# krullgit/3D-Object-Detection-for-autonomous-navigation

Hardware: AMD Instinct MI355X
Metric: frames/sec (whole node) + p50 per-frame ms, 16k-pt pillars (higher is better)
Workload: dtype f32 (GEMMs on the 16-bit matrix pipe as split operands -- two float16 pieces per value, 3 products, fp32 accumulate: fp32-equivalent results, measured 1.5e-6 max from the fp32 oracle at this shape)

## Files before the change

### 3d-object-detection-for-autonomous-navigation_amd/csrc/pfn.hip

```cpp
#include <stdlib.h>

#include "pp_common.h"
#include "anchor_mask_dev.h"

template <int N>
struct FVec { float v[N]; };

__device__ __forceinline__ float bcast(float x, int srclane) {
    return __int_as_float(__builtin_amdgcn_readlane(__float_as_int(x), srclane));
}

__device__ __forceinline__ float raw_max(float a, float b) {
    float r;
    asm("v_max_f32 %0, %1, %2" : "=v"(r) : "v"(a), "v"(b));
    return r;
}

__device__ __forceinline__ float wave_sum(float x) {
#pragma unroll
    for (int off = 32; off >= 1; off >>= 1) x += __shfl_xor(x, off);
    return x;
}

#define PFN_CW 4
template <int CPL, int F, bool PADDED, bool DIST = false>
__global__ __launch_bounds__(256) void k_pfn_canvas(PfnParams p) {
    constexpr int FA = F + 5 + (DIST ? 1 : 0);
    const int lane = threadIdx.x & 63, wave = threadIdx.x >> 6;
    const int b = blockIdx.y;
    const int ncanvas = p.ny * p.nx;
    const int cell0 = (blockIdx.x * 4 + wave) * PFN_CW;
    if (cell0 >= ncanvas) return;
    const int ncells = min(PFN_CW, ncanvas - cell0);
    const int C = p.C;
    const int ch0 = lane * CPL;
    const bool ch_ok = ch0 < C;

    float w[FA][CPL], bias[CPL];
#pragma unroll
    for (int k = 0; k < FA; ++k)
#pragma unroll
        for (int q = 0; q < CPL; ++q) w[k][q] = ch_ok ? p.w[k * C + ch0 + q] : 0.f;
#pragma unroll
    for (int q = 0; q < CPL; ++q) bias[q] = ch_ok ? p.bias[ch0 + q] : 0.f;
    float wsx[CPL], wsy[CPL], wsz[CPL];
#pragma unroll
    for (int q = 0; q < CPL; ++q) {
        wsx[q] = (w[0][q] + w[F + 0][q]) + w[F + 3][q];
        wsy[q] = (w[1][q] + w[F + 1][q]) + w[F + 4][q];
        wsz[q] = w[2][q] + w[F + 2][q];
    }

    const int* map = p.cellmap + (size_t)b * p.nz * ncanvas;
    unsigned occ = 0;
    for (int z = 0; z < p.nz; ++z) {
        const int v = (lane < ncells) ? map[(size_t)z * ncanvas + cell0 + lane] : -1;
        occ |= (unsigned)(__ballot(v >= 0) & ((1ull << PFN_CW) - 1ull));
    }

    float* cbase = p.canvas + ((size_t)b * ncanvas + cell0) * C;
    {
        const int nq = ncells * C / 4;
        const float4 z4 = make_float4(0.f, 0.f, 0.f, 0.f);
        for (int q = lane; q < nq; q += 64) {
            const int c = (q * 4) / C;
            if (!((occ >> c) & 1u)) reinterpret_cast<float4*>(cbase)[q] = z4;
        }
    }

    const int n0 = PADDED ? 0 : p.offsets[b];
    const int* ps = PADDED ? nullptr : p.pillar_start + (size_t)b * (p.max_voxels + 1);
    const int T = p.T;

    while (occ) {
        const int c = __builtin_ctz(occ);
        occ &= occ - 1;
        const int cell = cell0 + c;
        const int yi = cell / p.nx, xi = cell - yi * p.nx;
        const float cxf = __fadd_rn(__fmul_rn((float)xi, p.vx), p.x_off);
        const float cyf = __fadd_rn(__fmul_rn((float)yi, p.vy), p.y_off);
        float acc[CPL];
#pragma unroll
        for (int q = 0; q < CPL; ++q) acc[q] = 0.f;

        for (int z = 0; z < p.nz; ++z) {
            const int pid = __builtin_amdgcn_readfirstlane(map[(size_t)z * ncanvas + cell]);
            if (pid < 0) continue;
            int n, nsum;
            const float* src;
            if (PADDED) {
                n = __builtin_amdgcn_readfirstlane(min(max(p.num_points[pid], 0), T));
                nsum = T;
                src = p.voxels + (size_t)pid * T * F;
            } else {
                const int start = __builtin_amdgcn_readfirstlane(ps[pid]);
                n = __builtin_amdgcn_readfirstlane(min(ps[pid + 1] - start, T));
                nsum = n;
                src = p.pts_sorted + (size_t)(n0 + start) * F;
            }
            float sx = 0.f, sy = 0.f, sz = 0.f;
            for (int j0 = 0; j0 < nsum; j0 += 64) {
                const int j = j0 + lane;
                if (j < nsum) {
                    const float* q = src + (size_t)j * F;
                    sx += q[0]; sy += q[1]; sz += q[2];
                }
            }
            sx = wave_sum(sx); sy = wave_sum(sy); sz = wave_sum(sz);
            const float fn = (float)n;
            const float mx = sx / fn, my = sy / fn, mz = sz / fn;

            const float dxm = mx - cxf, dym = my - cyf;
            float kp[CPL], m[CPL];
#pragma unroll
            for (int q = 0; q < CPL; ++q) {
                float k0 = bias[q];
                k0 = fmaf(cxf, w[0][q], k0);
                k0 = fmaf(cyf, w[1][q], k0);
                k0 = fmaf(-dxm, w[F + 0][q], k0);
                k0 = fmaf(-dym, w[F + 1][q], k0);
                k0 = fmaf(-mz, w[F + 2][q], k0);
                kp[q] = k0;
                m[q] = -3.0e38f;
            }
            for (int j0 = 0; j0 < n; j0 += 64) {
                const int j = j0 + lane;
                float pt[F];
#pragma unroll
                for (int f = 0; f < F; ++f) pt[f] = 0.f;
                if (j < n) {
                    const float* q = src + (size_t)j * F;
#pragma unroll
                    for (int f = 0; f < F; ++f) pt[f] = q[f];
                }
                float pdist = 0.f;
                if (DIST) pdist = __fsqrt_rn(__fadd_rn(__fadd_rn(__fmul_rn(pt[0], pt[0]), __fmul_rn(pt[1], pt[1])), __fmul_rn(pt[2], pt[2])));
                pt[0] = pt[0] - cxf;
                pt[1] = pt[1] - cyf;
                const int cnt = min(64, n - j0);
                for (int jj = 0; jj < cnt; ++jj) {
                    float ft[F];
#pragma unroll
                    for (int f = 0; f < F; ++f) ft[f] = bcast(pt[f], jj);
                    const float fd = DIST ? bcast(pdist, jj) : 0.f;
#pragma unroll
                    for (int q = 0; q < CPL; ++q) {
                        float o = kp[q];
                        o = fmaf(ft[0], wsx[q], o);
                        o = fmaf(ft[1], wsy[q], o);
                        o = fmaf(ft[2], wsz[q], o);
                        if (F > 3) o = fmaf(ft[F - 1], w[F - 1][q], o);
                        if (DIST) o = fmaf(fd, w[FA - 1][q], o);
                        m[q] = fmaxf(m[q], o);
                    }
                }
            }
#pragma unroll
            for (int q = 0; q < CPL; ++q) m[q] = fmaxf(m[q], 0.f);
            if (n < T) {
#pragma unroll
                for (int q = 0; q < CPL; ++q) m[q] = fmaxf(m[q], fmaxf(bias[q], 0.f));
            }
            if (p.feat_out != nullptr && ch_ok) {
                const size_t row = PADDED ? (size_t)pid : ((size_t)b * p.max_voxels + pid);
#pragma unroll
                for (int q = 0; q < CPL; ++q) p.feat_out[row * C + ch0 + q] = m[q];
            }
#pragma unroll
            for (int q = 0; q < CPL; ++q) acc[q] += m[q];
        }
        if (ch_ok) {
            float* dst = cbase + (size_t)c * C + ch0;
            if constexpr (CPL == 4) {
                *reinterpret_cast<float4*>(dst) = make_float4(acc[0], acc[1], acc[2], acc[3]);
            } else if constexpr (CPL == 2) {
                *reinterpret_cast<float2*>(dst) = make_float2(acc[0], acc[1]);
            } else {
                dst[0] = acc[0];
            }
        }
    }
}

#ifndef PFN2_CW
#define PFN2_CW 8
#endif
template <int CPL, int F, bool PIL = false>
__global__ __launch_bounds__(256) void k_pfn_canvas2(PfnParams p) {
    constexpr int FA = F + 5;
    const int lane = threadIdx.x & 63, wave = threadIdx.x >> 6;
    const int b = blockIdx.y;
    const int ncanvas = p.ny * p.nx;
    const int amb = (p.am_mask != nullptr) ? AM_PFN_BLOCKS : 0;
    if ((int)blockIdx.x < amb) {
        extern __shared__ int sI[];
        const int part = (int)blockIdx.x;
        const int64_t per = (p.am_A + AM_PFN_BLOCKS - 1) / AM_PFN_BLOCKS;
        const int64_t a0 = part * per, a1 = (a0 + per < p.am_A) ? a0 + per : p.am_A;
        anchor_mask_frame_block<256>(p.cellmap + (size_t)b * p.nz * ncanvas, p.nz, p.ny, p.nx, p.am_cells, a0, a1,
                                     p.am_threshold, p.am_mask + (size_t)b * p.am_A, sI);
        return;
    }
    const int bx = (int)blockIdx.x - amb;
    const int NW = PIL ? 1 : ((int)gridDim.x - amb) * 4;
    const int wid = PIL ? (bx * 4 + wave) * PFN2_CW : bx * 4 + wave;
    const int np_frame = PIL ? p.npillars[b] : 0;
    if (PIL ? (wid >= np_frame) : (wid >= ncanvas)) return;
    const int ncells = PIL ? min(PFN2_CW, np_frame - wid) : min(PFN2_CW, (ncanvas - wid + NW - 1) / NW);
    const int nz = p.nz;
    const int NS = ncells * nz;
    const int C = p.C, T = p.T;
    const int ch0 = lane * CPL;
    const bool ch_ok = ch0 < C;

    const int n0 = p.offsets[b];
    const int* ps = p.pillar_start + (size_t)b * (p.max_voxels + 1);
    int pid = -1, start = 0, cnt = 0, slot_cell = 0;
    float slot_cx = 0.f, slot_cy = 0.f;
    [[maybe_unused]] int col_xy = 0;
    if constexpr (PIL) {
        int z0 = 0;
        bool primary = false;
        if (lane < ncells) {
            const int cz = p.pillar_cell[(size_t)b * p.max_voxels + wid + lane];
            z0 = cz / ncanvas;
            col_xy = cz - z0 * ncanvas;
            primary = true;
            for (int z = 0; z < z0; ++z) primary = primary & (p.cellmap[((size_t)b * nz + z) * ncanvas + col_xy] < 0);
            if (p.occbits != nullptr) {
                const int yy = col_xy / p.nx, xx = col_xy - yy * p.nx;
                atomicOr(p.occbits + ((size_t)b * p.ny + yy) * occ_words(p.nx) + ((xx + 1) >> 6), 1ull << ((xx + 1) & 63));
            }
        }
        if (lane < NS) {
            const int c = lane / nz, z = lane - c * nz;
            slot_cell = c;
            const int cxy = __shfl(col_xy, c), zc = __shfl(z0, c);
            const bool prim = __shfl((int)primary, c) != 0;
            if (prim && z == zc) pid = wid + c;
            else if (prim && z > zc) pid = p.cellmap[((size_t)b * nz + z) * ncanvas + cxy];
        }
    } else {
        if (lane < NS) {
            const int c = lane / nz, z = lane - c * nz;
            slot_cell = c;
            pid = p.cellmap[((size_t)b * nz + z) * ncanvas + wid + c * NW];
        }
    }
    if (PIL && __ballot(pid >= 0) == 0ull) return;
    if (lane < NS) {
        const int c = slot_cell;
        if (pid >= 0) {
            start = ps[pid];
            cnt = min(ps[pid + 1] - start, T);
        }
        const int cell = PIL ? __shfl(col_xy, c) : wid + c * NW;
        const int yi = cell / p.nx, xi = cell - yi * p.nx;
        slot_cx = __fadd_rn(__fmul_rn((float)xi, p.vx), p.x_off);
        slot_cy = __fadd_rn(__fmul_rn((float)yi, p.vy), p.y_off);
    }
    float w[FA][CPL], bias[CPL];
#pragma unroll
    for (int k = 0; k < FA; ++k)
#pragma unroll
        for (int q = 0; q < CPL; ++q) w[k][q] = ch_ok ? p.w[k * C + ch0 + q] : 0.f;
#pragma unroll
    for (int q = 0; q < CPL; ++q) bias[q] = ch_ok ? p.bias[ch0 + q] : 0.f;
    float wsx[CPL], wsy[CPL], wsz[CPL];
#pragma unroll
    for (int q = 0; q < CPL; ++q) {
        wsx[q] = (w[0][q] + w[F + 0][q]) + w[F + 3][q];
        wsy[q] = (w[1][q] + w[F + 1][q]) + w[F + 4][q];
        wsz[q] = w[2][q] + w[F + 2][q];
    }

    const int incl = wave_inclusive_scan(cnt);
    const int excl = incl - cnt;
    const int tot = __builtin_amdgcn_readlane(incl, 63);
    if (PIL && tot == 0) return;
    const float* src = p.pts_sorted + (size_t)n0 * F;

    struct Batch { int slot; float x, y, z, i; };
    auto load_batch = [&](int base) -> Batch {
        Batch r;
        r.slot = -1; r.x = r.y = r.z = r.i = 0.f;
        const int g = base + lane;
        int sl = 0;
        for (int s = 0; s < NS; ++s) sl += (g >= __builtin_amdgcn_readlane(incl, s)) ? 1 : 0;
        sl = min(sl, NS - 1);
        const int st = __shfl(start, sl), ex = __shfl(excl, sl);
        const float pcx = __shfl(slot_cx, sl), pcy = __shfl(slot_cy, sl);
        if (g < tot) {
            r.slot = sl;
            const float* q = src + (size_t)(st + (g - ex)) * F;
            r.x = q[0] - pcx;
            r.y = q[1] - pcy;
            r.z = q[2];
            if (F > 3) r.i = q[F - 1];
        }
        return r;
    };

    float* cbase = p.canvas + ((size_t)b * ncanvas + (PIL ? 0 : wid)) * C;
    const size_t cstep = (size_t)NW * C;
    float acc[CPL], m[CPL];
#pragma unroll
    for (int q = 0; q < CPL; ++q) { acc[q] = 0.f; m[q] = -3.0e38f; }
    int cur_slot = -1, cur_cell = 0;
    float cxf = 0.f, cyf = 0.f, sx = 0.f, sy = 0.f, sz = 0.f;
    bool cell_dirty = false;
    auto write_cell = [&](int c) {
        if (ch_ok && (cell_dirty || !PIL)) {
            float* dst = PIL ? cbase + (size_t)__builtin_amdgcn_readlane(col_xy, c) * C + ch0 : cbase + (size_t)c * cstep + ch0;
            if constexpr (CPL == 4) *reinterpret_cast<float4*>(dst) = make_float4(acc[0], acc[1], acc[2], acc[3]);
            else if constexpr (CPL == 2) *reinterpret_cast<float2*>(dst) = make_float2(acc[0], acc[1]);
            else dst[0] = acc[0];
        }
#pragma unroll
        for (int q = 0; q < CPL; ++q) acc[q] = 0.f;
        cell_dirty = false;
    };
    auto finish_slot = [&](int s) {
        const int n = __builtin_amdgcn_readlane(cnt, s);
        const float rn = __builtin_amdgcn_rcpf((float)n);
        const float dxm = sx * rn, dym = sy * rn, mz = sz * rn;
#pragma unroll
        for (int q = 0; q < CPL; ++q) {
            float k0 = bias[q];
            k0 = fmaf(cxf, w[0][q], k0);
            k0 = fmaf(cyf, w[1][q], k0);
            k0 = fmaf(-dxm, w[F + 0][q], k0);
            k0 = fmaf(-dym, w[F + 1][q], k0);
            k0 = fmaf(-mz, w[F + 2][q], k0);
            m[q] = fmaxf(k0 + m[q], 0.f);
        }
        if (n < T) {
#pragma unroll
            for (int q = 0; q < CPL; ++q) m[q] = fmaxf(m[q], fmaxf(bias[q], 0.f));
        }
        if (p.feat_out != nullptr && ch_ok) {
            const size_t row = (size_t)b * p.max_voxels + __builtin_amdgcn_readlane(pid, s);
#pragma unroll
            for (int q = 0; q < CPL; ++q) p.feat_out[row * C + ch0 + q] = m[q];
        }
#pragma unroll
        for (int q = 0; q < CPL; ++q) { acc[q] += m[q]; m[q] = -3.0e38f; }
        cell_dirty = true;
    };
    auto begin_slot = [&](int s) {
        const int c = __builtin_amdgcn_readlane(slot_cell, s);
        while (cur_cell < c) { write_cell(cur_cell); ++cur_cell; }
        cxf = bcast(slot_cx, s);
        cyf = bcast(slot_cy, s);
        sx = sy = sz = 0.f;
        cur_slot = s;
    };
    Batch cur = load_batch(0);
    int left = 0;
    int next_slot = 0;
    for (int base = 0; base < tot; base += 64) {
        Batch nxt = cur;
        if (base + 64 < tot) nxt = load_batch(base + 64);
        const int nb = min(64, tot - base);
        for (int jj = 0; jj < nb; ++jj) {
            if (left == 0) {
                if (cur_slot >= 0) finish_slot(cur_slot);
                while ((left = __builtin_amdgcn_readlane(cnt, next_slot)) == 0) ++next_slot;
                begin_slot(next_slot);
                ++next_slot;
            }
            --left;
            const float fx = bcast(cur.x, jj), fy = bcast(cur.y, jj), fz = bcast(cur.z, jj);
            const float fi = (F > 3) ? bcast(cur.i, jj) : 0.f;
            sx += fx; sy += fy; sz += fz;
            if constexpr (CPL == 2) {
                typedef float f32x2 __attribute__((ext_vector_type(2)));
                const f32x2 vx = {fx, fx}, vy = {fy, fy}, vz = {fz, fz};
                const f32x2 wx2 = {wsx[0], wsx[1]}, wy2 = {wsy[0], wsy[1]}, wz2 = {wsz[0], wsz[1]};
                f32x2 o = vx * wx2;
                o = __builtin_elementwise_fma(vy, wy2, o);
                o = __builtin_elementwise_fma(vz, wz2, o);
                if (F > 3) {
                    const f32x2 vi = {fi, fi}, wi2 = {w[F - 1][0], w[F - 1][1]};
                    o = __builtin_elementwise_fma(vi, wi2, o);
                }
                m[0] = raw_max(m[0], o.x);
                m[1] = raw_max(m[1], o.y);
            } else {
#pragma unroll
                for (int q = 0; q < CPL; ++q) {
                    float o = fx * wsx[q];
                    o = fmaf(fy, wsy[q], o);
                    o = fmaf(fz, wsz[q], o);
                    if (F > 3) o = fmaf(fi, w[F - 1][q], o);
                    m[q] = raw_max(m[q], o);
                }
            }
        }
        cur = nxt;
    }
    if (cur_slot >= 0) finish_slot(cur_slot);
    while (cur_cell < ncells) { write_cell(cur_cell); ++cur_cell; }
}

static bool pfn_first_generation();
bool pfn_can_carry_anchor_mask(const PfnParams& p, bool padded_source) {
    return !padded_source && p.feat_out == nullptr && PFN2_CW * p.nz <= 64 && !pfn_first_generation() && !p.sparse &&
           p.ny * (p.nx | 1) <= AM_MAX_CELLS && !p.with_distance;
}
static bool pfn_first_generation() {
    static int v = -1;
    if (v < 0) {
        const char* e = getenv("PP_PFN_KERNEL");
        v = (e && e[0] == '1') ? 1 : 0;
    }
    return v == 1;
}

static bool pfn_pillar_centric(const PfnParams& p, bool padded) {
    return !padded && !p.with_distance && p.sparse && p.pillar_cell != nullptr && p.npillars != nullptr && PFN2_CW * p.nz <= 64 &&
           !pfn_first_generation();
}
bool pfn_writes_occbits(const PfnParams& p, bool padded) { return pfn_pillar_centric(p, padded); }

template <int CPL, int F>
static void launch_pfn_t(const PfnParams& p, bool padded, hipStream_t s) {
    const int ncanvas = p.ny * p.nx;
    dim3 grid((ncanvas + 4 * PFN_CW - 1) / (4 * PFN_CW), p.batch);
    if (p.with_distance) {
        if (padded) PP_LAUNCH("k_pfn_canvas", (k_pfn_canvas<CPL, F, true, true>), grid, dim3(256), 0, s, p);
        else PP_LAUNCH("k_pfn_canvas", (k_pfn_canvas<CPL, F, false, true>), grid, dim3(256), 0, s, p);
    } else if (padded) {
        PP_LAUNCH("k_pfn_canvas", (k_pfn_canvas<CPL, F, true>), grid, dim3(256), 0, s, p);
    } else if (pfn_pillar_centric(p, padded)) {
        dim3 gridp((p.max_voxels + 4 * PFN2_CW - 1) / (4 * PFN2_CW), p.batch);
        PP_LAUNCH("k_pfn_canvas2", (k_pfn_canvas2<CPL, F, true>), gridp, dim3(256), 0, s, p);
    } else if (PFN2_CW * p.nz <= 64 && !pfn_first_generation()) {
        dim3 grid2((ncanvas + 4 * PFN2_CW - 1) / (4 * PFN2_CW) + (p.am_mask != nullptr ? AM_PFN_BLOCKS : 0), p.batch);
        const size_t lds = (p.am_mask != nullptr) ? (size_t)p.ny * (p.nx | 1) * sizeof(int) : 0;
        PP_LAUNCH("k_pfn_canvas2", (k_pfn_canvas2<CPL, F>), grid2, dim3(256), lds, s, p);
    } else {
        PP_LAUNCH("k_pfn_canvas", (k_pfn_canvas<CPL, F, false>), grid, dim3(256), 0, s, p);
    }
}

int launch_pfn(const PfnParams& p, bool padded, hipStream_t s) {
    if (p.batch <= 0) return 0;
    const int C = p.C;
    int cpl;
    if (C <= 64) cpl = 1;
    else if (C == 128) cpl = 2;
    else if (C == 256) cpl = 4;
    else return PP_ERR_UNSUPPORTED;
    if (C % 4 != 0) return PP_ERR_UNSUPPORTED;
    if (p.F != 3 && p.F != 4) return PP_ERR_UNSUPPORTED;
#define PFN_CASE(CPLV, FV) \
    if (cpl == CPLV && p.F == FV) { launch_pfn_t<CPLV, FV>(p, padded, s); return 0; }
    PFN_CASE(1, 3) PFN_CASE(1, 4) PFN_CASE(2, 3) PFN_CASE(2, 4) PFN_CASE(4, 3) PFN_CASE(4, 4)
#undef PFN_CASE
    return PP_ERR_UNSUPPORTED;
}
```

Baseline: 90520.

## Stage point batches in LDS and precompute per-slot means in parallel

Each wave now writes its 64-point batch into a per-wave LDS ring and reads points back from LDS instead of broadcasting four registers per point with readlane. Per-slot coordinate sums and means are computed in parallel, one lane per slot, and stored in an LDS record, which removes the serial per-point accumulation. The inner loop is restructured around a ballot mask of slot-end positions and processes points two at a time between slot boundaries. This adds LDS usage (12 KB per block), which can lower occupancy, and adds wave barriers per batch.

```diff
diff --git a/3d-object-detection-for-autonomous-navigation_amd/csrc/pfn.hip b/3d-object-detection-for-autonomous-navigation_amd/csrc/pfn.hip
--- a/3d-object-detection-for-autonomous-navigation_amd/csrc/pfn.hip
+++ b/3d-object-detection-for-autonomous-navigation_amd/csrc/pfn.hip
@@ -185,6 +185,8 @@
 #ifndef PFN2_CW
 #define PFN2_CW 8
 #endif
+#define PFN2_LDS_WAVE (64 + 2 * 64)
+static constexpr size_t kPfn2Lds = 4 * PFN2_LDS_WAVE * sizeof(float4);
 template <int CPL, int F, bool PIL = false>
 __global__ __launch_bounds__(256) void k_pfn_canvas2(PfnParams p) {
     constexpr int FA = F + 5;
@@ -280,19 +282,20 @@
     if (PIL && tot == 0) return;
     const float* src = p.pts_sorted + (size_t)n0 * F;
 
-    struct Batch { int slot; float x, y, z, i; };
+    struct Batch { float x, y, z, i; int last; };
     auto load_batch = [&](int base) -> Batch {
         Batch r;
-        r.slot = -1; r.x = r.y = r.z = r.i = 0.f;
+        r.x = r.y = r.z = r.i = 0.f;
+        r.last = 0;
         const int g = base + lane;
         int sl = 0;
         for (int s = 0; s < NS; ++s) sl += (g >= __builtin_amdgcn_readlane(incl, s)) ? 1 : 0;
         sl = min(sl, NS - 1);
-        const int st = __shfl(start, sl), ex = __shfl(excl, sl);
+        const int off = __shfl(start - excl, sl), ic = __shfl(incl, sl);
         const float pcx = __shfl(slot_cx, sl), pcy = __shfl(slot_cy, sl);
         if (g < tot) {
-            r.slot = sl;
-            const float* q = src + (size_t)(st + (g - ex)) * F;
+            r.last = (g + 1 == ic) ? 1 : 0;
+            const float* q = src + (size_t)(off + g) * F;
             r.x = q[0] - pcx;
             r.y = q[1] - pcy;
             r.z = q[2];
@@ -301,13 +304,16 @@
         return r;
     };
 
+    extern __shared__ float4 sPfn[];
+    float4* ring = sPfn + __builtin_amdgcn_readfirstlane(wave) * PFN2_LDS_WAVE;
+    float4* srec = ring + 64;
+
     float* cbase = p.canvas + ((size_t)b * ncanvas + (PIL ? 0 : wid)) * C;
     const size_t cstep = (size_t)NW * C;
     float acc[CPL], m[CPL];
 #pragma unroll
     for (int q = 0; q < CPL; ++q) { acc[q] = 0.f; m[q] = -3.0e38f; }
-    int cur_slot = -1, cur_cell = 0;
-    float cxf = 0.f, cyf = 0.f, sx = 0.f, sy = 0.f, sz = 0.f;
+    int cur_cell = 0;
     bool cell_dirty = false;
     auto write_cell = [&](int c) {
         if (ch_ok && (cell_dirty || !PIL)) {
@@ -321,9 +327,11 @@
         cell_dirty = false;
     };
     auto finish_slot = [&](int s) {
+        const int c = __builtin_amdgcn_readlane(slot_cell, s);
+        while (cur_cell < c) { write_cell(cur_cell); ++cur_cell; }
         const int n = __builtin_amdgcn_readlane(cnt, s);
-        const float rn = __builtin_amdgcn_rcpf((float)n);
-        const float dxm = sx * rn, dym = sy * rn, mz = sz * rn;
+        const float4 sr = srec[2 * s];
+        const float cxf = sr.x, cyf = sr.y, dxm = sr.z, dym = sr.w, mz = srec[2 * s + 1].x;
 #pragma unroll
         for (int q = 0; q < CPL; ++q) {
             float k0 = bias[q];
@@ -347,59 +355,77 @@
         for (int q = 0; q < CPL; ++q) { acc[q] += m[q]; m[q] = -3.0e38f; }
         cell_dirty = true;
     };
-    auto begin_slot = [&](int s) {
-        const int c = __builtin_amdgcn_readlane(slot_cell, s);
-        while (cur_cell < c) { write_cell(cur_cell); ++cur_cell; }
-        cxf = bcast(slot_cx, s);
-        cyf = bcast(slot_cy, s);
-        sx = sy = sz = 0.f;
-        cur_slot = s;
+    auto point = [&](const float4 r) {
+        const float fx = r.x, fy = r.y, fz = r.z, fi = r.w;
+        if constexpr (CPL == 2) {
+            typedef float f32x2 __attribute__((ext_vector_type(2)));
+            const f32x2 vx = {fx, fx}, vy = {fy, fy}, vz = {fz, fz};
+            const f32x2 wx2 = {wsx[0], wsx[1]}, wy2 = {wsy[0], wsy[1]}, wz2 = {wsz[0], wsz[1]};
+            f32x2 o = vx * wx2;
+            o = __builtin_elementwise_fma(vy, wy2, o);
+            o = __builtin_elementwise_fma(vz, wz2, o);
+            if (F > 3) {
+                const f32x2 vi = {fi, fi}, wi2 = {w[F - 1][0], w[F - 1][1]};
+                o = __builtin_elementwise_fma(vi, wi2, o);
+            }
+            m[0] = raw_max(m[0], o.x);
+            m[1] = raw_max(m[1], o.y);
+        } else {
+#pragma unroll
+            for (int q = 0; q < CPL; ++q) {
+                float o = fx * wsx[q];
+                o = fmaf(fy, wsy[q], o);
+                o = fmaf(fz, wsz[q], o);
+                if (F > 3) o = fmaf(fi, w[F - 1][q], o);
+                m[q] = raw_max(m[q], o);
+            }
+        }
     };
+    float ssx = 0.f, ssy = 0.f, ssz = 0.f;
+    unsigned long long todo = __ballot(cnt > 0);
     Batch cur = load_batch(0);
-    int left = 0;
-    int next_slot = 0;
     for (int base = 0; base < tot; base += 64) {
         Batch nxt = cur;
         if (base + 64 < tot) nxt = load_batch(base + 64);
         const int nb = min(64, tot - base);
-        for (int jj = 0; jj < nb; ++jj) {
-            if (left == 0) {
-                if (cur_slot >= 0) finish_slot(cur_slot);
-                while ((left = __builtin_amdgcn_readlane(cnt, next_slot)) == 0) ++next_slot;
-                begin_slot(next_slot);
-                ++next_slot;
-            }
-            --left;
-            const float fx = bcast(cur.x, jj), fy = bcast(cur.y, jj), fz = bcast(cur.z, jj);
-            const float fi = (F > 3) ? bcast(cur.i, jj) : 0.f;
-            sx += fx; sy += fy; sz += fz;
-            if constexpr (CPL == 2) {
-                typedef float f32x2 __attribute__((ext_vector_type(2)));
-                const f32x2 vx = {fx, fx}, vy = {fy, fy}, vz = {fz, fz};
-                const f32x2 wx2 = {wsx[0], wsx[1]}, wy2 = {wsy[0], wsy[1]}, wz2 = {wsz[0], wsz[1]};
-                f32x2 o = vx * wx2;
-                o = __builtin_elementwise_fma(vy, wy2, o);
-                o = __builtin_elementwise_fma(vz, wz2, o);
-                if (F > 3) {
-                    const f32x2 vi = {fi, fi}, wi2 = {w[F - 1][0], w[F - 1][1]};
-                    o = __builtin_elementwise_fma(vi, wi2, o);
-                }
-                m[0] = raw_max(m[0], o.x);
-                m[1] = raw_max(m[1], o.y);
-            } else {
-#pragma unroll
-                for (int q = 0; q < CPL; ++q) {
-                    float o = fx * wsx[q];
-                    o = fmaf(fy, wsy[q], o);
-                    o = fmaf(fz, wsz[q], o);
-                    if (F > 3) o = fmaf(fi, w[F - 1][q], o);
-                    m[q] = raw_max(m[q], o);
-                }
+        ring[lane] = make_float4(cur.x, cur.y, cur.z, cur.i);
+        unsigned long long ends = __ballot(cur.last != 0);
+        __builtin_amdgcn_fence(__ATOMIC_RELEASE, "wavefront");
+        __builtin_amdgcn_wave_barrier();
+        __builtin_amdgcn_fence(__ATOMIC_ACQUIRE, "wavefront");
+        if (cnt > 0) {
+            const int lo = max(excl - base, 0), hi = min(incl - base, nb);
+            for (int j = lo; j < hi; ++j) {
+                const float4 r = ring[j];
+                ssx += r.x; ssy += r.y; ssz += r.z;
+            }
+            if (incl > base && incl - base <= nb) {
+                const float rn = __builtin_amdgcn_rcpf((float)cnt);
+                srec[2 * lane] = make_float4(slot_cx, slot_cy, ssx * rn, ssy * rn);
+                srec[2 * lane + 1].x = ssz * rn;
+            }
+        }
+        __builtin_amdgcn_fence(__ATOMIC_RELEASE, "wavefront");
+        __builtin_amdgcn_wave_barrier();
+        __builtin_amdgcn_fence(__ATOMIC_ACQUIRE, "wavefront");
+        int j = 0;
+        while (j < nb) {
+            const int e = ends ? (int)__builtin_ctzll(ends) : nb - 1;
+            for (; j < e; j += 2) {
+                const float4 r0 = ring[j], r1 = ring[j + 1];
+                point(r0);
+                point(r1);
+            }
+            if (j == e) point(ring[j++]);
+            if (ends) {
+                ends &= ends - 1;
+                const int s = (int)__builtin_ctzll(todo);
+                todo &= todo - 1;
+                finish_slot(s);
             }
         }
         cur = nxt;
     }
-    if (cur_slot >= 0) finish_slot(cur_slot);
     while (cur_cell < ncells) { write_cell(cur_cell); ++cur_cell; }
 }
 
@@ -434,10 +460,11 @@
         PP_LAUNCH("k_pfn_canvas", (k_pfn_canvas<CPL, F, true>), grid, dim3(256), 0, s, p);
     } else if (pfn_pillar_centric(p, padded)) {
         dim3 gridp((p.max_voxels + 4 * PFN2_CW - 1) / (4 * PFN2_CW), p.batch);
-        PP_LAUNCH("k_pfn_canvas2", (k_pfn_canvas2<CPL, F, true>), gridp, dim3(256), 0, s, p);
+        PP_LAUNCH("k_pfn_canvas2", (k_pfn_canvas2<CPL, F, true>), gridp, dim3(256), kPfn2Lds, s, p);
     } else if (PFN2_CW * p.nz <= 64 && !pfn_first_generation()) {
         dim3 grid2((ncanvas + 4 * PFN2_CW - 1) / (4 * PFN2_CW) + (p.am_mask != nullptr ? AM_PFN_BLOCKS : 0), p.batch);
-        const size_t lds = (p.am_mask != nullptr) ? (size_t)p.ny * (p.nx | 1) * sizeof(int) : 0;
+        const size_t am_lds = (p.am_mask != nullptr) ? (size_t)p.ny * (p.nx | 1) * sizeof(int) : 0;
+        const size_t lds = am_lds > kPfn2Lds ? am_lds : kPfn2Lds;
         PP_LAUNCH("k_pfn_canvas2", (k_pfn_canvas2<CPL, F>), grid2, dim3(256), lds, s, p);
     } else {
         PP_LAUNCH("k_pfn_canvas", (k_pfn_canvas<CPL, F, false>), grid, dim3(256), 0, s, p);
```

Result: no change. 90930, median of 4 (+0.4%).
